# sloisel/LinearAlgebraMPI.jl

Hardware: AMD Instinct MI355X
Metric: SpMV GFLOP/s (2*nnz/t), 2-D 5-pt Poisson, fp64 (higher is better)
Workload: dtype f64

## Files before the change

include/hpcla_rocm.h:

```cpp
#ifndef HPCLA_ROCM_H
#define HPCLA_ROCM_H

#include <stdint.h>

#ifdef __cplusplus
extern "C" {
#endif

#define HPCLA_VERSION 100

#define HPCLA_OK 0
#define HPCLA_ERR_INVALID -1
#define HPCLA_ERR_HIP -2
#define HPCLA_ERR_RCCL -3
#define HPCLA_ERR_NO_DEVICE -4
#define HPCLA_ERR_UNSUPPORTED -5
#define HPCLA_ERR_ALLOC -6

#define HPCLA_LAYOUT_ROW 0
#define HPCLA_LAYOUT_COL 1

typedef struct hpcla_comm hpcla_comm_t;
typedef struct hpcla_halo_plan hpcla_halo_plan_t;

// ... 332 lines not shown
int64_t hpcla_cols16_padded_len(int64_t nnz);
int hpcla_cols16_encode_i32(const int32_t *rowptr, const int32_t *colval_split, int64_t nrows, int64_t nnz, int64_t n_own,
                            int index_base, const int32_t *block_list, int64_t n_blocks, int16_t *cols16,
                            int *ineligible_dev, void *stream);
int hpcla_spmv_cols16_f64_i32(const int32_t *rowptr, const int16_t *cols16, const double *nzval, const double *x, double *y,
                              int64_t nrows, int64_t nnz, int index_base, const int32_t *block_list, int64_t n_blocks,
                              void *stream);
int hpcla_spmv_dist_cols16_f64_i32(hpcla_halo_plan_t *plan, const int32_t *rowptr, const int32_t *colval_split,
                                   const int16_t *cols16, const double *nzval, const double *x, int64_t n_own, double *y,
                                   int64_t nrows, int64_t nnz, int index_base, const int32_t *interior_blocks,
                                   int64_t n_interior, const int32_t *boundary_blocks, int64_t n_boundary, void *stream);
int hpcla_spmv_dist_dot_cols16_f64_i32(hpcla_halo_plan_t *plan, hpcla_comm_t *comm, const int32_t *rowptr,
                                       const int32_t *colval_split, const int16_t *cols16, const double *nzval,
                                       const double *x, int64_t n_own, double *y, int64_t nrows, int64_t nnz,
                                       int index_base, const int32_t *interior_blocks, int64_t n_interior,
                                       const int32_t *boundary_blocks, int64_t n_boundary, double *dot_out_dev,
                                       void *work, void *stream);
int hpcla_spmv_tune_block_order_cols16_f64_i32(const int32_t *rowptr, const int16_t *cols16, const double *nzval,
                                               const double *x_own, double *y_scratch, int64_t nrows, int64_t nnz,
                                               int index_base, int64_t block_base, int64_t n_blocks, void *stream,
                                               int *chosen_group);

#define HPCLA_BLOCK_PATTERNS_WEAK_HASH 1
typedef struct hpcla_block_patterns hpcla_block_patterns_t;
int hpcla_block_patterns_create_i32(hpcla_block_patterns_t **out, const int32_t *rowptr, const int16_t *cols16, int64_t nrows,
                                    int64_t nnz, int index_base, const int32_t *block_list, int64_t block_base,
                                    int64_t n_blocks, int flags, void *stream);
int hpcla_block_patterns_destroy(hpcla_block_patterns_t *p);
int hpcla_block_patterns_info(const hpcla_block_patterns_t *p, int64_t *n_patterns, int64_t *table_bytes,
                              int64_t *n_candidates, int64_t *n_patterned);
int hpcla_spmv_patterns_f64_i32(const int32_t *rowptr, const int16_t *cols16, const hpcla_block_patterns_t *patterns,
                                const double *nzval, const double *x, double *y, int64_t nrows, int64_t nnz, int index_base,
                                const int32_t *block_list, int64_t n_blocks, void *stream);
int hpcla_spmv_dist_patterns_f64_i32(hpcla_halo_plan_t *plan, const int32_t *rowptr, const int32_t *colval_split,
                                     const int16_t *cols16, const hpcla_block_patterns_t *patterns, const double *nzval,
                                     const double *x, int64_t n_own, double *y, int64_t nrows, int64_t nnz, int index_base,
                                     const int32_t *interior_blocks, int64_t n_interior, const int32_t *boundary_blocks,
                                     int64_t n_boundary, void *stream);
int hpcla_spmv_dist_dot_patterns_f64_i32(hpcla_halo_plan_t *plan, hpcla_comm_t *comm, const int32_t *rowptr,
                                         const int32_t *colval_split, const int16_t *cols16,
                                         const hpcla_block_patterns_t *patterns, const double *nzval, const double *x,
                                         int64_t n_own, double *y, int64_t nrows, int64_t nnz, int index_base,
                                         const int32_t *interior_blocks, int64_t n_interior,
                                         const int32_t *boundary_blocks, int64_t n_boundary, double *dot_out_dev, void *work,
                                         void *stream);
int hpcla_spmv_tune_block_order_patterns_f64_i32(const int32_t *rowptr, const int16_t *cols16,
                                                 const hpcla_block_patterns_t *patterns, const double *nzval,
                                                 const double *x_own, double *y_scratch, int64_t nrows, int64_t nnz,
                                                 int index_base, int64_t block_base, int64_t n_blocks, void *stream,
                                                 int *chosen_group);

typedef struct hpcla_packed hpcla_packed_t;
int hpcla_packed_create_i32(hpcla_packed_t **out, const int32_t *rowptr, const int32_t *colval_split,
// ... 176 lines not shown
```

linearalgebrampi.jl_amd/_capi.py:

```python
from __future__ import annotations

import ctypes
import os

_HERE = os.path.dirname(os.path.abspath(__file__))
LIB_PATH = os.path.join(_HERE, "libhpcla_rocm.so")

OK = 0
LAYOUT_ROW = 0
LAYOUT_COL = 1
UNIQUE_ID_BYTES = 128
WINDOW_DESC_BYTES = 128
WINDOW_TABLE_ROWS = 4
COMM_NO_RCCL = 1
HALO_SINGLE_BUFFER = 1
BLOCK_PATTERNS_WEAK_HASH = 1


class HPCLAError(RuntimeError):
    def __init__(self, fn: str, status: int, text: str):
        super().__init__(f"{fn} failed with status {status}: {text}")
        self.status = status


_lib = None

_i32 = ctypes.c_int
_i64 = ctypes.c_int64
_u64 = ctypes.c_uint64
_f64 = ctypes.c_double
_f32 = ctypes.c_float
_vp = ctypes.c_void_p

_SIGNATURES = {
    "hpcla_version": [],
    "hpcla_last_error": [],
    "hpcla_device_count": [_vp],
    "hpcla_set_device": [_i32],
    "hpcla_device_info": [_i32, _vp, _vp, _i32],
    "hpcla_spmv_csr_f64_i32": [_vp, _vp, _vp, _vp, _vp, _i64, _i64, _i32, _vp],
    "hpcla_spmv_csr_f64_i64": [_vp, _vp, _vp, _vp, _vp, _i64, _i64, _i32, _vp],
    "hpcla_spmv_split_f64_i32": [_vp, _vp, _vp, _vp, _vp, _i64, _vp, _i64, _i64, _i32, _vp, _i64, _vp],
    "hpcla_spmv_split_f64_i64": [_vp, _vp, _vp, _vp, _vp, _i64, _vp, _i64, _i64, _i32, _vp, _i64, _vp],
    "hpcla_spmv_rows_per_block": [],
    "hpcla_spmv_longrows_work_bytes": [_i64],
    "hpcla_spmv_longrows_f64_i32": [_vp, _vp, _vp, _vp, _vp, _i64, _vp, _i64, _i64, _i32, _vp, _i64, _i64, _vp, _vp],
    "hpcla_spmv_longrows_f64_i64": [_vp, _vp, _vp, _vp, _vp, _i64, _vp, _i64, _i64, _i32, _vp, _i64, _i64, _vp, _vp],
    "hpcla_spmv_block_order_hint": [_vp, _i32],
    "hpcla_spmv_tune_block_order_f64_i32": [_vp, _vp, _vp, _vp, _vp, _i64, _vp, _i64, _i64, _i32, _vp, _vp],
    "hpcla_spmv_tune_block_order_f64_i64": [_vp, _vp, _vp, _vp, _vp, _i64, _vp, _i64, _i64, _i32, _vp, _vp],
    "hpcla_spmv_tune_block_order_cols16_f64_i32": [_vp, _vp, _vp, _vp, _vp, _i64, _i64, _i32, _i64, _i64, _vp, _vp],
    "hpcla_cols16_padded_len": [_i64],
    "hpcla_cols16_encode_i32": [_vp, _vp, _i64, _i64, _i64, _i32, _vp, _i64, _vp, _vp, _vp],
    "hpcla_spmv_cols16_f64_i32": [_vp, _vp, _vp, _vp, _vp, _i64, _i64, _i32, _vp, _i64, _vp],
    "hpcla_block_patterns_create_i32": [_vp, _vp, _vp, _i64, _i64, _i32, _vp, _i64, _i64, _i32, _vp],
    "hpcla_block_patterns_destroy": [_vp],
    "hpcla_block_patterns_info": [_vp, _vp, _vp, _vp, _vp],
    "hpcla_spmv_patterns_f64_i32": [_vp, _vp, _vp, _vp, _vp, _vp, _i64, _i64, _i32, _vp, _i64, _vp],
    "hpcla_spmv_tune_block_order_patterns_f64_i32": [_vp, _vp, _vp, _vp, _vp, _vp, _i64, _i64, _i32, _i64, _i64, _vp, _vp],
    "hpcla_spmm_rows_per_block": [],
    "hpcla_spmm_runs_desc_bytes": [_i64],
    "hpcla_spmm_runs_build_i32": [_vp, _vp, _i64, _i64, _i32, _i64, _vp, _vp, _vp],
    "hpcla_spmm_runs_build_i64": [_vp, _vp, _i64, _i64, _i32, _i64, _vp, _vp, _vp],
    "hpcla_spmm_banded_blocks_i32": [_vp, _vp, _i64, _i64, _i32, _i64, _i32, _vp, _vp],
    "hpcla_spmm_banded_blocks_i64": [_vp, _vp, _i64, _i64, _i32, _i64, _i32, _vp, _vp],
    "hpcla_spmm_runs_k16_f64_i32": [_vp, _vp, _vp, _vp, _vp, _i64, _vp, _i64, _i64, _i32, _vp, _vp, _i64, _vp],
    "hpcla_spmm_runs_k16_f64_i64": [_vp, _vp, _vp, _vp, _vp, _i64, _vp, _i64, _i64, _i32, _vp, _vp, _i64, _vp],
    "hpcla_spmm_runs_colmajor_k16_f64_i32": [_vp, _vp, _vp, _vp, _i64, _vp, _i64, _i64, _vp, _i64, _i64, _i64, _i32, _vp, _vp, _i64, _vp],
    "hpcla_spmm_runs_colmajor_k16_f64_i64": [_vp, _vp, _vp, _vp, _i64, _vp, _i64, _i64, _vp, _i64, _i64, _i64, _i32, _vp, _vp, _i64, _vp],
    "hpcla_spmm_runs_colmajor_tune_block_order_f64_i32": [_vp, _vp, _vp, _vp, _i64, _vp, _i64, _i64, _vp, _i64, _i64, _i64, _i32, _vp, _vp, _i64, _vp, _vp],
    "hpcla_spmm_runs_colmajor_tune_block_order_f64_i64": [_vp, _vp, _vp, _vp, _i64, _vp, _i64, _i64, _vp, _i64, _i64, _i64, _i32, _vp, _vp, _i64, _vp, _vp],
    "hpcla_spmm_block_order_hint": [_vp, _i32],
    "hpcla_spmm_tune_block_order_f64_i32": [_vp, _vp, _vp, _vp, _i64, _vp, _i64, _i64, _vp, _i64, _i64, _i64, _i32, _i32,
                                            _vp, _i64, _vp, _vp],
    "hpcla_spmm_tune_block_order_f64_i64": [_vp, _vp, _vp, _vp, _i64, _vp, _i64, _i64, _vp, _i64, _i64, _i64, _i32, _i32,
                                            _vp, _i64, _vp, _vp],
    "hpcla_remap_i32": [_vp, _vp, _vp, _i64, _i32, _vp],
    "hpcla_remap_i64": [_vp, _vp, _vp, _i64, _i32, _vp],
    "hpcla_remap_i64_to_i32": [_vp, _vp, _vp, _i64, _i32, _vp],
    "hpcla_narrow_i64_to_i32": [_vp, _vp, _i64, _vp, _vp],
# ... 224 lines not shown
```

linearalgebrampi.jl_amd/csrc/patterns.h:

```cpp
#pragma once
#include "common.h"

namespace hpcla {

constexpr int PAT_RPB = 256;
constexpr int PAT_HEAD = 272;
constexpr int PAT_NR = 257, PAT_PHASE = 258, PAT_WAVE = 260;
constexpr int64_t PAT_TABLE_CAP_BYTES = 256 * 1024;
constexpr int64_t PAT_MAX_LEN = 65535;

struct alignas(8) PatRec {
    int32_t first;
    int32_t id;
};

struct PatArgs {
    const PatRec *rec;
    const int16_t *table;
};

}

struct hpcla_block_patterns {
    int64_t nrows = 0, nnz = 0, all_blocks = 0;
    int index_base = 0;
    hpcla::PatRec *rec = nullptr;
    int16_t *table = nullptr;
    int64_t table_bytes = 0, n_patterns = 0, n_candidates = 0, n_patterned = 0;
};
```

linearalgebrampi.jl_amd/csrc/patterns.hip:

```cpp
#include <algorithm>
#include <unordered_map>
#include <vector>

#include "patterns.h"

namespace hpcla {

__device__ __forceinline__ uint64_t pat_mix(uint64_t key, uint64_t v)
{
    uint64_t z = key * 0x9E3779B97F4A7C15ull + v * 0xC2B2AE3D27D4EB4Full + 0x165667B19E3779F9ull;
    z = (z ^ (z >> 30)) * 0xBF58476D1CE4E5B9ull;
    z = (z ^ (z >> 27)) * 0x94D049BB133111EBull;
    return z ^ (z >> 31);
}

struct PatMeta {
    int32_t first, len;
};

__device__ __forceinline__ int64_t pat_block(const int32_t *list, int64_t base, int64_t b) { return list ? (int64_t)list[b] : base + b; }

__global__ __launch_bounds__(PAT_RPB) void pat_hash_kernel(const int32_t *__restrict__ rowptr, const int16_t *__restrict__ cols16,
                                                           int64_t nrows, int64_t nnz, int base, const int32_t *__restrict__ list,
                                                           int64_t run_base, int weak, uint64_t *__restrict__ hash,
// ... 51 lines not shown
                                                             PatRec *__restrict__ rec)
{
    const int64_t blk = pat_block(list, run_base, blockIdx.x);
    const PatRec rc = rec[blk];
    if (rc.id < 0) return;
    const int16_t *t = table + (int64_t)rc.id * 8;
    const int64_t r0 = blk * PAT_RPB;
    const int nr = (int)((nrows - r0) < PAT_RPB ? (nrows - r0) : PAT_RPB);
    const int64_t p0 = (int64_t)rowptr[r0] - base, len = (int64_t)rowptr[r0 + nr] - base - p0;
    const int phase = (int)(p0 & 7);
    int bad = (p0 != rc.first) | (t[PAT_NR] != (int16_t)nr) | (t[PAT_PHASE] != (int16_t)phase) | (len > PAT_MAX_LEN);
    if (!bad) {
        for (int i = threadIdx.x; i <= PAT_RPB; i += PAT_RPB)
            bad |= ((int64_t)(uint16_t)t[i] != (int64_t)rowptr[r0 + (i < nr ? i : nr)] - base - p0);
    }
    bad = __syncthreads_or(bad);
    if (!bad) {
        for (int64_t j = threadIdx.x; j < len; j += PAT_RPB) bad |= (t[PAT_HEAD + phase + j] != cols16[p0 + j]);
        bad = __syncthreads_or(bad);
    }
    if (bad && threadIdx.x == 0) rec[blk].id = -1;
}

static void patterns_free(hpcla_block_patterns *p)
{
    if (!p) return;
    if (p->rec) (void)hipFree(p->rec);
    if (p->table) (void)hipFree(p->table);
    delete p;
}

int patterns_args(const hpcla_block_patterns *p, int64_t nrows, int64_t nnz, int index_base, PatArgs *out)
{
    if (!p || !out) return set_error(HPCLA_ERR_INVALID, "block patterns: null handle");
    if (p->nrows != nrows || p->nnz != nnz || p->index_base != index_base)
        return set_error(HPCLA_ERR_INVALID, "block patterns: the handle was created for another structure (nrows / nnz / index_base)");
    out->rec = p->rec;
    out->table = p->table;
    return HPCLA_OK;
}

}

using namespace hpcla;

HPCLA_API int hpcla_block_patterns_create_i32(hpcla_block_patterns_t **out, const int32_t *rowptr, const int16_t *cols16,
                                              int64_t nrows, int64_t nnz, int index_base, const int32_t *block_list,
                                              int64_t block_base, int64_t n_blocks, int flags, void *stream)
{
    if (!out) return set_error(HPCLA_ERR_INVALID, "block_patterns_create: null out");
    *out = nullptr;
    if (nrows < 0 || nnz < 0) return set_error(HPCLA_ERR_INVALID, "block_patterns_create: negative size");
    if (index_base != 0 && index_base != 1) return set_error(HPCLA_ERR_INVALID, "block_patterns_create: index_base must be 0 or 1");
    if (flags & ~HPCLA_BLOCK_PATTERNS_WEAK_HASH) return set_error(HPCLA_ERR_INVALID, "block_patterns_create: unknown flag");
    const int64_t all_blocks = (nrows + PAT_RPB - 1) / PAT_RPB;
    int64_t nc = all_blocks, run_base = 0;
    if (block_list) {
        if (n_blocks < 0 || n_blocks > all_blocks) return set_error(HPCLA_ERR_INVALID, "block_patterns_create: n_blocks out of range");
        nc = n_blocks;
    } else if (block_base >= 0) {
        if (n_blocks < 0 || block_base + n_blocks > all_blocks)
            return set_error(HPCLA_ERR_INVALID, "block_patterns_create: block run out of bounds");
        nc = n_blocks;
        run_base = block_base;
    }
    if (nc == 0 || nnz == 0) return HPCLA_OK;
    if (!rowptr || !cols16) return set_error(HPCLA_ERR_INVALID, "block_patterns_create: null array");
    HPCLA_CHECK_GRID(nc, "block_patterns_create");
    hipStream_t s = as_stream(stream);

    uint64_t *d_hash = nullptr;
    PatMeta *d_meta = nullptr;
    PatRec *d_reps = nullptr;
    hpcla_block_patterns *p = nullptr;
    auto fail = [&](int code) {
        if (d_hash) (void)hipFree(d_hash);
        if (d_meta) (void)hipFree(d_meta);
        if (d_reps) (void)hipFree(d_reps);
        patterns_free(p);
        return code;
    };
#define PT_HIP(expr)                                                                                                   \
    do {                                                                                                               \
        hipError_t _e = (expr);                                                                                        \
        if (_e != hipSuccess) return fail(set_error(HPCLA_ERR_HIP, "%s failed: %s", #expr, hipGetErrorString(_e)));    \
    } while (0)
    PT_HIP(hipMalloc((void **)&d_hash, nc * sizeof(uint64_t)));
    PT_HIP(hipMalloc((void **)&d_meta, nc * sizeof(PatMeta)));
    pat_hash_kernel<<<(uint32_t)nc, PAT_RPB, 0, s>>>(rowptr, cols16, nrows, nnz, index_base, block_list, run_base,
                                                     (flags & HPCLA_BLOCK_PATTERNS_WEAK_HASH) ? 1 : 0, d_hash, d_meta);
    PT_HIP(hipGetLastError());
    std::vector<uint64_t> hash(nc);
    std::vector<PatMeta> meta(nc);
    std::vector<int32_t> blocks;
    PT_HIP(hipMemcpyAsync(hash.data(), d_hash, nc * sizeof(uint64_t), hipMemcpyDeviceToHost, s));
    PT_HIP(hipMemcpyAsync(meta.data(), d_meta, nc * sizeof(PatMeta), hipMemcpyDeviceToHost, s));
    if (block_list) {
        blocks.resize(nc);
// ... 34 lines not shown
    if (covered * 2 < nc || reps.empty()) return fail(HPCLA_OK);

    p = new hpcla_block_patterns;
    p->nrows = nrows; p->nnz = nnz; p->all_blocks = all_blocks; p->index_base = index_base;
    p->table_bytes = used * (int64_t)sizeof(int16_t);
    p->n_patterns = (int64_t)reps.size();
    p->n_candidates = nc;
    std::vector<PatRec> rec(all_blocks, PatRec{0, -1});
    for (int64_t b = 0; b < nc; ++b) {
        auto it = hash[b] == ~(uint64_t)0 ? kept.end() : kept.find(hash[b]);
        rec[block_of(b)] = PatRec{meta[b].first, it == kept.end() ? -1 : it->second};
    }
    PT_HIP(hipMalloc((void **)&p->rec, all_blocks * sizeof(PatRec)));
    PT_HIP(hipMalloc((void **)&p->table, p->table_bytes));
    PT_HIP(hipMalloc((void **)&d_reps, reps.size() * sizeof(PatRec)));
    PT_HIP(hipMemsetAsync(p->table, 0, p->table_bytes, s));
    PT_HIP(hipMemcpyAsync(p->rec, rec.data(), all_blocks * sizeof(PatRec), hipMemcpyHostToDevice, s));
    PT_HIP(hipMemcpyAsync(d_reps, reps.data(), reps.size() * sizeof(PatRec), hipMemcpyHostToDevice, s));
    pat_build_kernel<<<(uint32_t)reps.size(), PAT_RPB, 0, s>>>(rowptr, cols16, nrows, index_base, d_reps, p->table);
    PT_HIP(hipGetLastError());
    pat_verify_kernel<<<(uint32_t)nc, PAT_RPB, 0, s>>>(rowptr, cols16, nrows, index_base, block_list, run_base, p->table, p->rec);
    PT_HIP(hipGetLastError());
    PT_HIP(hipMemcpyAsync(rec.data(), p->rec, all_blocks * sizeof(PatRec), hipMemcpyDeviceToHost, s));
    PT_HIP(hipStreamSynchronize(s));
#undef PT_HIP
    for (const PatRec &r : rec) p->n_patterned += r.id >= 0;
    if (p->n_patterned * 2 < nc) return fail(HPCLA_OK);
    (void)hipFree(d_hash); (void)hipFree(d_meta); (void)hipFree(d_reps);
    *out = p;
    return HPCLA_OK;
}

HPCLA_API int hpcla_block_patterns_destroy(hpcla_block_patterns_t *p)
{
    patterns_free(p);
    return HPCLA_OK;
}

HPCLA_API int hpcla_block_patterns_info(const hpcla_block_patterns_t *p, int64_t *n_patterns, int64_t *table_bytes,
                                        int64_t *n_candidates, int64_t *n_patterned)
{
    if (!p) return set_error(HPCLA_ERR_INVALID, "block_patterns_info: null handle");
    if (n_patterns) *n_patterns = p->n_patterns;
    if (table_bytes) *table_bytes = p->table_bytes;
    if (n_candidates) *n_candidates = p->n_candidates;
    if (n_patterned) *n_patterned = p->n_patterned;
    return HPCLA_OK;
}
```

linearalgebrampi.jl_amd/csrc/spmv.hip:

```cpp
#include <stdlib.h>
#include <string.h>

#include <atomic>
#include <mutex>
#include <type_traits>
#include <unordered_map>

#include "common.h"
#include "halo_wait.h"
#include "patterns.h"

namespace hpcla {

constexpr int RPB = 256;
static_assert(RPB == PAT_RPB, "the pattern table is built for this kernel's row blocks");
constexpr int CHUNK = RPB * 8;
constexpr int UNROLL = CHUNK / RPB;

template <typename T, int N>
using vec = T __attribute__((ext_vector_type(N)));

struct Cols16 {};
struct Pat16 {};
template <typename P>
struct IndexPolicy {
    using row_t = P;
    using col_t = P;
    static constexpr int VEC = 4;
    static constexpr bool PATTERNS = false;
    static __device__ __forceinline__ int64_t decode(col_t c, int base, int64_t ) { return (int64_t)(P)(c - (P)base); }
    static __device__ __forceinline__ col_t fill(int base) { return (P)base; }
};
template <>
struct IndexPolicy<Cols16> {
    using row_t = int32_t;
    using col_t = int16_t;
    static constexpr int VEC = 8;
    static constexpr bool PATTERNS = false;
    static __device__ __forceinline__ int64_t decode(col_t d, int , int64_t r0) { return r0 + (int)d; }
    static __device__ __forceinline__ col_t fill(int ) { return 0; }
};
template <>
struct IndexPolicy<Pat16> : IndexPolicy<Cols16> {
    static constexpr bool PATTERNS = true;
};

template <bool SPLIT>
__device__ __forceinline__ double gather_x(const double *__restrict__ x_own,
                                           const double *__restrict__ x_ghost, int64_t n_own,
                                           int64_t col)
{
    if (SPLIT) {
        const double *p = col < n_own ? x_own + col : x_ghost + (col - n_own);
        return *p;
    }
    return x_own[col];
}

struct BlockSel {
    const int32_t *list;
    int64_t base;
    const int32_t *first_list;
    int64_t first_base;
    int64_t n_first;
    int64_t n_run;
    int32_t group_log2;
    int32_t nt_y;
// ... 18 lines not shown
            if (bs.first_list) return (int64_t)bs.first_list[b];
            return bs.first_base + (bs.group_log2 > 0 ? xcd_group_index(b, bs.n_run, bs.group_log2) : b);
        }
        wait = true;
        return bs.list ? (int64_t)bs.list[b - bs.n_first] : bs.base + (b - bs.n_first);
    }
    if (bs.list) return (int64_t)bs.list[b];
    return bs.base + (bs.group_log2 > 0 ? xcd_group_index(b, bs.n_run, bs.group_log2) : b);
}

__device__ __forceinline__ void block_dot_epilogue(double *s_scratch, double *__restrict__ dot_partial,
                                                   int64_t blk, double v)
{
#pragma unroll
    for (int off = 32; off > 0; off >>= 1) v += __shfl_down(v, off, 64);
    const int lane = threadIdx.x & 63, w = threadIdx.x >> 6;
    if (lane == 0) s_scratch[w] = v;
    __syncthreads();
    if (threadIdx.x == 0) dot_partial[blk] = ((s_scratch[0] + s_scratch[1]) + s_scratch[2]) + s_scratch[3];
}

constexpr int RG_CHW = 464;
constexpr int RG_UR = 8;

template <typename I, bool SPLIT, bool WAIT, bool LONGR = false>
__global__ __launch_bounds__(RPB) void spmv_rowgather_kernel(
    const typename IndexPolicy<I>::row_t *__restrict__ rowptr, const typename IndexPolicy<I>::col_t *__restrict__ colval,
    const double *__restrict__ nzval, const double *__restrict__ x_own, const double *x_ghost, int64_t n_own,
    double *__restrict__ y, int64_t nrows, int64_t nnz, int base,
    BlockSel bs, double *__restrict__ dot_partial, HaloWait hw, PushArgs push, int64_t long_min = 0, PatArgs pat = PatArgs{nullptr, nullptr})
{
    using IP = IndexPolicy<I>;
    using R = typename IP::row_t;
    using C = typename IP::col_t;
    constexpr int V = IP::VEC;
    constexpr int NV = (RG_CHW / V + 63) / 64;
    static_assert(!LONGR || !WAIT, "the long-row form is a plain launch");
    static_assert(V * sizeof(C) == 16 || sizeof(C) == 8, "one 16-byte column load per staged vector (Int64: two)");
    static_assert(RG_CHW % V == 0 && RG_CHW >= 64 * 7 + V - 1, "a pass holds a 7-entry stencil's wave behind any aligned start");
    __shared__ __attribute__((aligned(16))) C s_col_all[(RPB / 64) * RG_CHW];
    __shared__ __attribute__((aligned(16))) double s_val_all[(RPB / 64) * RG_CHW];
    __shared__ double s_red[RPB / 64];

    if constexpr (WAIT) {
        if ((int)blockIdx.x < push.n_blocks) {
            halo_push_block<R, RPB>(push, (int)blockIdx.x);
            return;
        }
    }
    const int tid = threadIdx.x;
    bool wait_ghosts;
    const int64_t blk = select_block<WAIT>(bs, wait_ghosts, WAIT ? push.n_blocks : 0);
    uint32_t waited = 0;
// ... 2 lines not shown
        x_ghost = hw.ghost0 + (int64_t)(waited & ~HALO_WAIT_TIMED_OUT) * hw.buf_stride;
    }
    const int64_t r0 = blk * RPB;
    const int nr = (int)((nrows - r0) < RPB ? (nrows - r0) : RPB);
    if (WAIT && (waited & HALO_WAIT_TIMED_OUT)) {
        if ((int)threadIdx.x < nr) y[r0 + threadIdx.x] = halo_poison();
        if (dot_partial && threadIdx.x == 0) dot_partial[blk] = halo_poison();
        return;
    }

    const int wave = __builtin_amdgcn_readfirstlane(tid >> 6), lane = tid & 63;
    C *s_col = s_col_all + wave * RG_CHW;
    double *s_val = s_val_all + wave * RG_CHW;
    const int64_t rw = r0 + wave * 64;
    const int nrw = nr - wave * 64 < 0 ? 0 : (nr - wave * 64 > 64 ? 64 : nr - wave * 64);
    double acc = 0.0, x_row = 0.0;
    if (nrw > 0) {
        const int ll = lane < nrw ? lane : nrw - 1;
        int64_t p0 = 0, p1 = 0;
        R rlo = 0, rhi = 0;
        const C *cols = colval;
        bool streamed = true;
        R roff = 0;
        if constexpr (IP::PATTERNS) {
            const int64_t rc64 = *reinterpret_cast<const int64_t *>(pat.rec + blk);
            const PatRec rc{(int32_t)rc64, (int32_t)(rc64 >> 32)};
            if (rc.id >= 0) {
                const int16_t *t = pat.table + (int64_t)rc.id * 8;
                const int32_t *wb = reinterpret_cast<const int32_t *>(t + PAT_WAVE) + wave;
                p0 = (int64_t)rc.first + wb[0];
                p1 = (int64_t)rc.first + wb[1];
                struct __attribute__((packed, aligned(2))) Pair { uint32_t v; };
                rlo = (R)reinterpret_cast<const Pair *>(t + wave * 64 + ll)->v;
                roff = rc.first + base;
                cols = t + PAT_HEAD - (rc.first & ~7);
                streamed = false;
            }
        }
        if (streamed) {
            p0 = (int64_t)rowptr[rw] - base;
            p1 = (int64_t)rowptr[rw + nrw] - base;
            rlo = rowptr[rw + ll];
            rhi = rowptr[rw + ll + 1];
        }
        const int64_t pa = p0 & ~(int64_t)(V - 1);
        const int64_t total = p1 - pa;
        if (dot_partial) x_row = x_own[rw + ll];
        const bool is_long = LONGR && lane < nrw && (int64_t)rhi - (int64_t)rlo >= long_min;
        for (int64_t c = 0; c < total; c += RG_CHW) {
            if (LONGR) {
                const int64_t lo_rel = (int64_t)rlo - base - pa, hi_rel = (int64_t)rhi - base - pa;
                const uint64_t covers = __ballot(is_long && lo_rel <= c && hi_rel >= c + RG_CHW);
                if (covers) {
                    const int64_t hi_l = __shfl(hi_rel, __ffsll((unsigned long long)covers) - 1, 64);
                    c = (hi_l / RG_CHW) * RG_CHW - RG_CHW;
                    continue;
                }
            }
            const int n = (int)((total - c) < RG_CHW ? (total - c) : RG_CHW);
            if (pa + c + ((n + V - 1) & ~(V - 1)) <= nnz) {
                const int last = (n - 1) & ~(V - 1);
                vec<C, V> cq[NV];
                vec<double, 2> va[NV][V / 2];
#pragma unroll
                for (int u = 0; u < NV; ++u) {
                    const int e0 = (u * 64 + lane) * V;
                    const int ee = e0 < last ? e0 : last;
                    cq[u] = *reinterpret_cast<const vec<C, V> *>(cols + pa + c + ee);
#pragma unroll
                    for (int k = 0; k < V / 2; ++k)
                        va[u][k] = *reinterpret_cast<const vec<double, 2> *>(nzval + pa + c + ee + 2 * k);
                }
// ... 315 lines not shown
    } else if (block_base >= 0) {
        if (n_blocks < 0 || block_base + n_blocks > all_blocks)
            return set_error(HPCLA_ERR_INVALID, "spmv: block range out of bounds");
        launch_blocks = n_blocks;
    } else {
        block_base = 0;
    }
    if (launch_blocks == 0) return HPCLA_OK;
    if (launch_blocks > 0x7fffffffLL) return set_error(HPCLA_ERR_INVALID, "spmv: too many blocks");
    dim3 grid((uint32_t)launch_blocks), block(RPB);
    hipStream_t s = as_stream(stream);
    if (split && !x_ghost) split = false;
    using IP = IndexPolicy<I>;
    const bool aligned = (reinterpret_cast<uintptr_t>(colval) % (IP::VEC * sizeof(typename IP::col_t)) == 0) &&
                         (reinterpret_cast<uintptr_t>(nzval) % 32 == 0);
    const BlockSel bs{block_list, block_base, nullptr, 0, 0, launch_blocks, block_list ? 0 : block_order_of(rowptr),
                      spmv_nt_y(dot_partial != nullptr)};
    HaloWait nowait;
    memset(&nowait, 0, sizeof(nowait));
    PushArgs nopush;
    memset(&nopush, 0, sizeof(nopush));
    if constexpr (std::is_same<I, Cols16>::value) {
        if (!aligned) return set_error(HPCLA_ERR_INVALID, "spmv: 16-bit columns need a 16-byte aligned copy and 32-byte aligned nzval");
        if (pat)
            spmv_rowgather_kernel<Pat16, false, false><<<grid, block, 0, s>>>(
                rowptr, colval, nzval, x_own, nullptr, 0, y, nrows, nnz, index_base, bs, dot_partial, nowait, nopush, 0, *pat);
        else
            spmv_rowgather_kernel<Cols16, false, false><<<grid, block, 0, s>>>(
                rowptr, colval, nzval, x_own, nullptr, 0, y, nrows, nnz, index_base, bs, dot_partial, nowait, nopush);
    } else if (aligned) {
        if (split)
            spmv_rowgather_kernel<I, true, false><<<grid, block, 0, s>>>(
                rowptr, colval, nzval, x_own, x_ghost, n_own, y, nrows, nnz, index_base, bs, dot_partial, nowait, nopush);
        else
            spmv_rowgather_kernel<I, false, false><<<grid, block, 0, s>>>(
                rowptr, colval, nzval, x_own, nullptr, 0, y, nrows, nnz, index_base, bs, dot_partial, nowait, nopush);
    } else {
        if (split)
            spmv_rowblock_kernel<I, true, false><<<grid, block, 0, s>>>(
                rowptr, colval, nzval, x_own, x_ghost, n_own, y, nrows, index_base, bs, dot_partial, nowait, nopush);
        else
            spmv_rowblock_kernel<I, false, false><<<grid, block, 0, s>>>(
                rowptr, colval, nzval, x_own, nullptr, 0, y, nrows, index_base, bs, dot_partial, nowait, nopush);
    }
    HPCLA_CHECK_LAUNCH();
    return HPCLA_OK;
}
// ... 118 lines not shown
                    double *dot_partial, int64_t block_base, const hpcla_block_patterns *patterns)
{
    PatArgs pa;
    if (patterns)
        if (const int rc = patterns_args(patterns, nrows, nnz, index_base, &pa)) return rc;
    return spmv_launch<Cols16>(rowptr, cols16, nzval, x, nullptr, 0, false, y, nrows, nnz, index_base, bl, nb, stream,
                               dot_partial, block_base, patterns ? &pa : nullptr);
}

}

using namespace hpcla;

HPCLA_API int hpcla_spmv_rows_per_block(void) { return RPB; }

static void set_block_order(const void *rowptr, int group_log2)
{
    std::lock_guard<std::mutex> lock(g_order_mu);
    if (group_log2 <= 0) g_order.erase(rowptr);
    else g_order[rowptr] = group_log2;
    g_order_count.store((int)g_order.size(), std::memory_order_relaxed);
}

template <typename I>
static int tune_block_order(const typename IndexPolicy<I>::row_t *rowptr, const typename IndexPolicy<I>::col_t *colval_split,
                            const double *nzval, const double *x_own,
                            const double *x_ghost, int64_t n_own, double *y_scratch, int64_t nrows, int64_t nnz,
                            int index_base, void *stream, int *chosen_group, int64_t run_base = -1, int64_t run_blocks = 0,
                            const PatArgs *pat = nullptr)
{
    if (chosen_group) *chosen_group = 1;
    if (nrows < 0 || nnz < 0 || !rowptr) return set_error(HPCLA_ERR_INVALID, "spmv_tune_block_order: bad arguments");
    set_block_order(rowptr, 0);
    const int64_t n_blocks = (nrows + RPB - 1) / RPB;
    if (n_blocks < 4096 || nnz == 0) return HPCLA_OK;
    if (run_base >= 0 && (run_blocks <= 0 || run_base + run_blocks > n_blocks))
        return run_blocks == 0 ? HPCLA_OK : set_error(HPCLA_ERR_INVALID, "spmv_tune_block_order: block run out of bounds");
    if (!y_scratch) return set_error(HPCLA_ERR_INVALID, "spmv_tune_block_order: null scratch vector");
    constexpr int NC = 4, ROUNDS = 4, REPS = 4;
    const int cand[NC] = {0, 3, 5, 6};
    float ms[NC][ROUNDS];
    hipEvent_t e0, e1;
    HPCLA_CHECK_HIP(hipEventCreate(&e0));
    HPCLA_CHECK_HIP(hipEventCreate(&e1));
    hipStream_t s = as_stream(stream);
    int rc = HPCLA_OK;
    for (int r = 0; r < ROUNDS && rc == HPCLA_OK; ++r)
        for (int c = 0; c < NC && rc == HPCLA_OK; ++c) {
            set_block_order(rowptr, cand[c]);
            if (hipEventRecord(e0, s) != hipSuccess) { rc = set_error(HPCLA_ERR_HIP, "spmv_tune_block_order: event"); break; }
            for (int i = 0; i < REPS && rc == HPCLA_OK; ++i)
                rc = spmv_launch<I>(rowptr, colval_split, nzval, x_own, x_ghost, n_own, true, y_scratch, nrows, nnz,
                                    index_base, nullptr, run_base >= 0 ? run_blocks : 0, stream, nullptr, run_base, pat);
            if (rc != HPCLA_OK) break;
            if (hipEventRecord(e1, s) != hipSuccess || hipEventSynchronize(e1) != hipSuccess ||
                hipEventElapsedTime(&ms[c][r], e0, e1) != hipSuccess)
                rc = set_error(HPCLA_ERR_HIP, "spmv_tune_block_order: timing");
        }
    (void)hipEventDestroy(e0);
    (void)hipEventDestroy(e1);
    set_block_order(rowptr, 0);
    if (rc != HPCLA_OK) return rc;
    float best_t[NC];
    for (int c = 0; c < NC; ++c) {
        float a = ms[c][1], b = ms[c][2], d = ms[c][3];
        best_t[c] = a > b ? (b > d ? b : (a > d ? d : a)) : (a > d ? a : (b > d ? d : b));
    }
    int best = 0;
    for (int c = 1; c < NC; ++c)
        if (best_t[c] < best_t[best]) best = c;
    if (best != 0 && best_t[best] > 0.99f * best_t[0]) best = 0;
    set_block_order(rowptr, cand[best]);
    if (chosen_group) *chosen_group = 1 << cand[best];
    return HPCLA_OK;
}

HPCLA_API int hpcla_spmv_tune_block_order_f64_i32(const int32_t *rowptr, const int32_t *colval_split, const double *nzval,
                                                  const double *x_own, const double *x_ghost, int64_t n_own,
                                                  double *y_scratch, int64_t nrows, int64_t nnz, int index_base,
                                                  void *stream, int *chosen_group)
{
    return tune_block_order<int32_t>(rowptr, colval_split, nzval, x_own, x_ghost, n_own, y_scratch, nrows, nnz, index_base,
                                     stream, chosen_group);
}

HPCLA_API int hpcla_spmv_tune_block_order_f64_i64(const int64_t *rowptr, const int64_t *colval_split, const double *nzval,
                                                  const double *x_own, const double *x_ghost, int64_t n_own,
                                                  double *y_scratch, int64_t nrows, int64_t nnz, int index_base,
                                                  void *stream, int *chosen_group)
{
    return tune_block_order<int64_t>(rowptr, colval_split, nzval, x_own, x_ghost, n_own, y_scratch, nrows, nnz, index_base,
                                     stream, chosen_group);
}

// ... 273 lines not shown
```

linearalgebrampi.jl_amd/sparse.py:

```python
from __future__ import annotations

import ctypes
from dataclasses import dataclass, field
from typing import Dict, List, Optional, Tuple

import numpy as np

from . import _capi
from .backends import (CommSerial, HPCBackend, assert_backends_compatible, attach_halo_windows, comm_allgather,
                       comm_alltoall_counts, comm_barrier, comm_exchange_indices, comm_rank, comm_size,
                       create_halo_plan, halo_ghost_ptr, halo_timed_out, require_device)
from .partition import (compute_partition_hash, compute_structural_hash, owner_of,
                        uniform_partition)
from .vectors import HPCVector, current_stream_ptr, dptr


import os as _os

_PACKED_BY_ENV = _os.environ.get("HPCLA_SPMV_PACKED", "") == "1"


def _torch():
    import torch
    return torch
# ... 101 lines not shown
            lo, hi = cut(cnt, c), cut(cnt, c + 1)
            chunk_of[off + lo:off + hi] = c
            newpos[off + lo:off + hi] = fill[c] + np.arange(hi - lo, dtype=np.int64)
            fill[c] += hi - lo
        off += cnt
    return send_chunks, recv_chunk_counts, chunk_of, newpos


INT32_MAX = int(np.iinfo(np.int32).max)


def narrowing_enabled() -> bool:
    return _os.environ.get("HPCLA_NARROW_INDICES", "1").strip().lower() not in ("0", "off", "false", "no")


def narrow_cols_enabled() -> bool:
    return _os.environ.get("HPCLA_NARROW_COLS", "1").strip().lower() not in ("0", "off", "false", "no")


def block_patterns_enabled() -> bool:
    return narrow_cols_enabled() and _os.environ.get("HPCLA_BLOCK_PATTERNS", "1").strip().lower() not in ("0", "off", "false", "no")


def create_block_patterns(rowptr_dev, cols16, nrows: int, nnz: int, block_list, block_base: int, n_blocks: int, flags: int = 0):
    h = ctypes.c_void_p()
    _capi.call("hpcla_block_patterns_create_i32", ctypes.byref(h), dptr(rowptr_dev), dptr(cols16), nrows, nnz, 0,
               dptr(block_list) if block_list is not None else None, block_base, n_blocks, flags, current_stream_ptr())
    return h if h else None


def block_patterns_info(handle) -> dict:
    v = [ctypes.c_int64() for _ in range(4)]
    _capi.call("hpcla_block_patterns_info", handle, *[ctypes.byref(c) for c in v])
    return dict(zip(("patterns", "table_bytes", "candidates", "patterned"), (int(c.value) for c in v)))


def encode_cols16(rowptr_dev, colval_split, nrows: int, nnz: int, n_own: int, block_list, n_blocks: int):
    torch = _torch()
    dev = colval_split.device
    out = torch.empty(_capi.load().hpcla_cols16_padded_len(nnz), dtype=torch.int16, device=dev)
    bad = torch.empty(1, dtype=torch.int32, device=dev)
    _capi.call("hpcla_cols16_encode_i32", dptr(rowptr_dev), dptr(colval_split), nrows, nnz, n_own, 0,
               dptr(block_list) if block_list is not None else None, n_blocks, dptr(out), dptr(bad), current_stream_ptr())
    return None if int(bad.item()) else out


def can_narrow_indices(nnz: int, nrows_local: int, n_own: int, n_ghost: int, index_base: int = 0) -> bool:
    lim = INT32_MAX - int(index_base)
    return (int(nnz) <= lim and int(nrows_local) <= lim and int(n_own) + int(n_ghost) <= lim and int(n_own) <= lim)


def split_colval(A: "HPCSparseMatrix", cmap: np.ndarray, to_i32: bool):
    torch = _torch()
    dev = A.backend.torch_device
    a64 = A.Ti == np.dtype(np.int64)
    out64 = a64 and not to_i32
    cmap_dev = torch.from_numpy(cmap.astype(np.int64 if out64 else np.int32)).to(dev)
# ... 57 lines not shown

        self.interior = self.boundary = None
        self.n_interior = self.n_boundary = 0
        if self.has_halo and A.nrows_local > 0:
            rpb = _capi.load().hpcla_spmv_rows_per_block()
            nblk = (A.nrows_local + rpb - 1) // rpb
            flags = torch.empty(nblk, dtype=torch.int32, device=dev)
            _capi.call(f"hpcla_classify_blocks_{sfx}", dptr(self.rowptr_of(A)), dptr(self.colval_split),
                       A.nrows_local, 0, self.n_own, rpb, dptr(flags), s)
            self.interior = torch.nonzero(flags == 0).flatten().to(torch.int32).contiguous()
            self.boundary = torch.nonzero(flags != 0).flatten().to(torch.int32).contiguous()
            self.n_interior = int(self.interior.numel())
            self.n_boundary = int(self.boundary.numel())
        self._keep = cmap_dev
        self.cols16 = None
        if (narrow_cols_enabled() and not self.is_i64 and not self.is_f32 and A.nrows_local > 0 and A.nnz > 0
                and (not self.has_halo or self.n_interior > 0)):
            self.cols16 = encode_cols16(self.rowptr_of(A), self.colval_split, A.nrows_local, A.nnz, self.n_own,
                                        self.interior if self.has_halo else None, self.n_interior if self.has_halo else 0)
        self.patterns = None
        if self.cols16 is not None and block_patterns_enabled():
            self.patterns = create_block_patterns(self.rowptr_of(A), self.cols16, A.nrows_local, A.nnz,
                                                  self.interior if self.has_halo else None, -1,
                                                  self.n_interior if self.has_halo else 0)
        self.block_group = 1
        self.block_group_measured = False
        want = _os.environ.get("HPCLA_BLOCK_ORDER", "auto").strip().lower()
        if want.isdigit():
            g = int(want)
            if g > 1024 or (g & (g - 1)) != 0:
                import sys
                sys.stderr.write(f"hpcla: HPCLA_BLOCK_ORDER={want} is not a power of two <= 1024; natural order\n")
                g = 1
            self.block_group = max(1, g)
        elif (want != "natural" and not self.is_f32 and A.nrows_local > 0 and A.nnz > 0
              and int(x.v.numel()) >= max(self.n_own, 1)):
            scratch = torch.empty(A.nrows_local, dtype=torch.float64, device=dev)
            ghost, _ng = self.ghost_tensor_ptr()
            chosen = ctypes.c_int(1)
            run = None
            if self.cols16 is not None and A.nzval.data_ptr() % 32 == 0:
                if not self.has_halo:
                    run = (-1, 0)
                else:
                    first, last = int(self.interior[0]), int(self.interior[-1])
                    if last - first + 1 == self.n_interior:
                        run = (first, self.n_interior)
# ... 36 lines not shown
    def timed_out(self) -> bool:
        return halo_timed_out(self.halo)

    def destroy(self) -> None:
        if getattr(self, "patterns", None) is not None:
            _capi.call("hpcla_block_patterns_destroy", self.patterns)
            self.patterns = None
        if self.halo:
            _capi.call("hpcla_halo_plan_destroy", self.halo)
            self.halo = ctypes.c_void_p()


_vector_plan_cache: Dict[tuple, VectorPlan] = {}


def get_vector_plan(A: "HPCSparseMatrix", x: HPCVector) -> VectorPlan:
    key = (A._ensure_hash(), x.structural_hash, str(A.T), str(A.Ti), "ROCArray")
    if A.Ti == np.dtype(np.int64) and not narrowing_enabled():
        key += ("wide",)
    if not narrow_cols_enabled():
        key += ("cols32",)
    elif not block_patterns_enabled():
        key += ("nopat",)
    plan = _vector_plan_cache.get(key)
    if plan is None:
        plan = VectorPlan(A, x)
        plan.key = key
        _vector_plan_cache[key] = plan
    if getattr(plan if plan.narrowed else A, "_block_order_hint", 1) != plan.block_group:
        _hint_block_order(A, plan)
    A._block_order_hint = plan.block_group
    return plan


def _unhint_block_order(ptr: int) -> None:
    try:
        _capi.load().hpcla_spmv_block_order_hint(ctypes.c_void_p(ptr), 0)
    except Exception:
        pass


def _unhint_spmm_block_order(ptr: int) -> None:
    try:
        _capi.load().hpcla_spmm_block_order_hint(ctypes.c_void_p(ptr), 0)
    except Exception:
        pass
# ... 510 lines not shown
```

Measured before the change: 1014.

## Add per-row column records for short block patterns in SpMV row-gather

```diff
diff --git a/include/hpcla_rocm.h b/include/hpcla_rocm.h
--- a/include/hpcla_rocm.h
+++ b/include/hpcla_rocm.h
@@ -378,6 +378,7 @@
                                                int *chosen_group);
 
 #define HPCLA_BLOCK_PATTERNS_WEAK_HASH 1
+#define HPCLA_BLOCK_PATTERNS_NO_ROWS 2
 typedef struct hpcla_block_patterns hpcla_block_patterns_t;
 int hpcla_block_patterns_create_i32(hpcla_block_patterns_t **out, const int32_t *rowptr, const int16_t *cols16, int64_t nrows,
                                     int64_t nnz, int index_base, const int32_t *block_list, int64_t block_base,
@@ -385,6 +386,7 @@
 int hpcla_block_patterns_destroy(hpcla_block_patterns_t *p);
 int hpcla_block_patterns_info(const hpcla_block_patterns_t *p, int64_t *n_patterns, int64_t *table_bytes,
                               int64_t *n_candidates, int64_t *n_patterned);
+int hpcla_block_patterns_rows_info(const hpcla_block_patterns_t *p, int64_t *n_row_patterns, int64_t *row_bytes);
 int hpcla_spmv_patterns_f64_i32(const int32_t *rowptr, const int16_t *cols16, const hpcla_block_patterns_t *patterns,
                                 const double *nzval, const double *x, double *y, int64_t nrows, int64_t nnz, int index_base,
                                 const int32_t *block_list, int64_t n_blocks, void *stream);
diff --git a/linearalgebrampi.jl_amd/_capi.py b/linearalgebrampi.jl_amd/_capi.py
--- a/linearalgebrampi.jl_amd/_capi.py
+++ b/linearalgebrampi.jl_amd/_capi.py
@@ -15,6 +15,7 @@
 COMM_NO_RCCL = 1
 HALO_SINGLE_BUFFER = 1
 BLOCK_PATTERNS_WEAK_HASH = 1
+BLOCK_PATTERNS_NO_ROWS = 2
 
 
 class HPCLAError(RuntimeError):
@@ -56,6 +57,7 @@
     "hpcla_block_patterns_create_i32": [_vp, _vp, _vp, _i64, _i64, _i32, _vp, _i64, _i64, _i32, _vp],
     "hpcla_block_patterns_destroy": [_vp],
     "hpcla_block_patterns_info": [_vp, _vp, _vp, _vp, _vp],
+    "hpcla_block_patterns_rows_info": [_vp, _vp, _vp],
     "hpcla_spmv_patterns_f64_i32": [_vp, _vp, _vp, _vp, _vp, _vp, _i64, _i64, _i32, _vp, _i64, _vp],
     "hpcla_spmv_tune_block_order_patterns_f64_i32": [_vp, _vp, _vp, _vp, _vp, _vp, _i64, _i64, _i32, _i64, _i64, _vp, _vp],
     "hpcla_spmm_rows_per_block": [],
diff --git a/linearalgebrampi.jl_amd/csrc/patterns.h b/linearalgebrampi.jl_amd/csrc/patterns.h
--- a/linearalgebrampi.jl_amd/csrc/patterns.h
+++ b/linearalgebrampi.jl_amd/csrc/patterns.h
@@ -5,9 +5,13 @@
 
 constexpr int PAT_RPB = 256;
 constexpr int PAT_HEAD = 272;
-constexpr int PAT_NR = 257, PAT_PHASE = 258, PAT_WAVE = 260;
+constexpr int PAT_NR = 257, PAT_PHASE = 258, PAT_WAVE = 260, PAT_ROWS = 270;
 constexpr int64_t PAT_TABLE_CAP_BYTES = 256 * 1024;
 constexpr int64_t PAT_MAX_LEN = 65535;
+constexpr int PAT_ROW_K = 8;
+constexpr int PAT_PASS = 464;
+constexpr int64_t PAT_ROWS_PATTERN_BYTES = (int64_t)PAT_RPB * PAT_ROW_K * 2;
+constexpr int64_t PAT_ROWS_CAP_BYTES = 256 * 1024;
 
 struct alignas(8) PatRec {
     int32_t first;
@@ -17,6 +21,7 @@
 struct PatArgs {
     const PatRec *rec;
     const int16_t *table;
+    const int16_t *rows;
 };
 
 }
@@ -26,5 +31,7 @@
     int index_base = 0;
     hpcla::PatRec *rec = nullptr;
     int16_t *table = nullptr;
+    int16_t *rows = nullptr;
+    int64_t n_row_patterns = 0;
     int64_t table_bytes = 0, n_patterns = 0, n_candidates = 0, n_patterned = 0;
 };
diff --git a/linearalgebrampi.jl_amd/csrc/patterns.hip b/linearalgebrampi.jl_amd/csrc/patterns.hip
--- a/linearalgebrampi.jl_amd/csrc/patterns.hip
+++ b/linearalgebrampi.jl_amd/csrc/patterns.hip
@@ -97,9 +97,35 @@
     if (bad && threadIdx.x == 0) rec[blk].id = -1;
 }
 
+__global__ __launch_bounds__(PAT_RPB) void pat_rows_kernel(int16_t *__restrict__ table, const int32_t *__restrict__ place,
+                                                           const int32_t *__restrict__ which, int16_t *__restrict__ rows)
+{
+    const int32_t w = which[blockIdx.x];
+    if (w < 0) return;
+    int16_t *t = table + (int64_t)place[blockIdx.x] * 8;
+    const int i = threadIdx.x, nr = t[PAT_NR], phase = t[PAT_PHASE];
+    const int lo = (uint16_t)t[i], hi = (uint16_t)t[i + 1];
+    int16_t *r = rows + ((int64_t)w * PAT_RPB + i) * PAT_ROW_K;
+#pragma unroll
+    for (int u = 0; u < PAT_ROW_K; ++u) r[u] = (i < nr && lo + u < hi) ? t[PAT_HEAD + phase + lo + u] : (int16_t)0;
+    if (i == 0) *reinterpret_cast<int32_t *>(t + PAT_ROWS) = w + 1;
+}
+
+static bool pattern_is_short(const int16_t *t)
+{
+    const int phase = t[PAT_PHASE];
+    for (int i = 0; i < PAT_RPB; ++i)
+        if ((int)(uint16_t)t[i + 1] - (int)(uint16_t)t[i] > PAT_ROW_K) return false;
+    const int32_t *wb = reinterpret_cast<const int32_t *>(t + PAT_WAVE);
+    for (int w = 0; w < PAT_RPB / 64; ++w)
+        if (((wb[w] + phase) & 7) + (wb[w + 1] - wb[w]) > PAT_PASS) return false;
+    return true;
+}
+
 static void patterns_free(hpcla_block_patterns *p)
 {
     if (!p) return;
+    if (p->rows) (void)hipFree(p->rows);
     if (p->rec) (void)hipFree(p->rec);
     if (p->table) (void)hipFree(p->table);
     delete p;
@@ -112,6 +138,7 @@
         return set_error(HPCLA_ERR_INVALID, "block patterns: the handle was created for another structure (nrows / nnz / index_base)");
     out->rec = p->rec;
     out->table = p->table;
+    out->rows = p->rows;
     return HPCLA_OK;
 }
 
@@ -127,7 +154,7 @@
     *out = nullptr;
     if (nrows < 0 || nnz < 0) return set_error(HPCLA_ERR_INVALID, "block_patterns_create: negative size");
     if (index_base != 0 && index_base != 1) return set_error(HPCLA_ERR_INVALID, "block_patterns_create: index_base must be 0 or 1");
-    if (flags & ~HPCLA_BLOCK_PATTERNS_WEAK_HASH) return set_error(HPCLA_ERR_INVALID, "block_patterns_create: unknown flag");
+    if (flags & ~(HPCLA_BLOCK_PATTERNS_WEAK_HASH | HPCLA_BLOCK_PATTERNS_NO_ROWS)) return set_error(HPCLA_ERR_INVALID, "block_patterns_create: unknown flag");
     const int64_t all_blocks = (nrows + PAT_RPB - 1) / PAT_RPB;
     int64_t nc = all_blocks, run_base = 0;
     if (block_list) {
@@ -147,8 +174,10 @@
     uint64_t *d_hash = nullptr;
     PatMeta *d_meta = nullptr;
     PatRec *d_reps = nullptr;
+    int32_t *d_which = nullptr;
     hpcla_block_patterns *p = nullptr;
     auto fail = [&](int code) {
+        if (d_which) (void)hipFree(d_which);
         if (d_hash) (void)hipFree(d_hash);
         if (d_meta) (void)hipFree(d_meta);
         if (d_reps) (void)hipFree(d_reps);
@@ -229,11 +258,34 @@
     pat_verify_kernel<<<(uint32_t)nc, PAT_RPB, 0, s>>>(rowptr, cols16, nrows, index_base, block_list, run_base, p->table, p->rec);
     PT_HIP(hipGetLastError());
     PT_HIP(hipMemcpyAsync(rec.data(), p->rec, all_blocks * sizeof(PatRec), hipMemcpyDeviceToHost, s));
+    std::vector<int16_t> table;
+    if (!(flags & HPCLA_BLOCK_PATTERNS_NO_ROWS)) {
+        table.resize(used);
+        PT_HIP(hipMemcpyAsync(table.data(), p->table, p->table_bytes, hipMemcpyDeviceToHost, s));
+    }
     PT_HIP(hipStreamSynchronize(s));
-#undef PT_HIP
     for (const PatRec &r : rec) p->n_patterned += r.id >= 0;
     if (p->n_patterned * 2 < nc) return fail(HPCLA_OK);
+    if (!(flags & HPCLA_BLOCK_PATTERNS_NO_ROWS)) {
+        std::vector<int32_t> pw(2 * reps.size());
+        for (size_t k = 0; k < reps.size(); ++k) {
+            pw[k] = reps[k].id;
+            const bool take = (p->n_row_patterns + 1) * PAT_ROWS_PATTERN_BYTES <= PAT_ROWS_CAP_BYTES &&
+                              pattern_is_short(table.data() + (int64_t)reps[k].id * 8);
+            pw[reps.size() + k] = take ? (int32_t)p->n_row_patterns++ : -1;
+        }
+        if (p->n_row_patterns > 0) {
+            PT_HIP(hipMalloc((void **)&p->rows, p->n_row_patterns * PAT_ROWS_PATTERN_BYTES));
+            PT_HIP(hipMalloc((void **)&d_which, pw.size() * sizeof(int32_t)));
+            PT_HIP(hipMemcpyAsync(d_which, pw.data(), pw.size() * sizeof(int32_t), hipMemcpyHostToDevice, s));
+            pat_rows_kernel<<<(uint32_t)reps.size(), PAT_RPB, 0, s>>>(p->table, d_which, d_which + reps.size(), p->rows);
+            PT_HIP(hipGetLastError());
+            PT_HIP(hipStreamSynchronize(s));
+        }
+    }
+#undef PT_HIP
     (void)hipFree(d_hash); (void)hipFree(d_meta); (void)hipFree(d_reps);
+    if (d_which) (void)hipFree(d_which);
     *out = p;
     return HPCLA_OK;
 }
@@ -254,3 +306,11 @@
     if (n_patterned) *n_patterned = p->n_patterned;
     return HPCLA_OK;
 }
+
+HPCLA_API int hpcla_block_patterns_rows_info(const hpcla_block_patterns_t *p, int64_t *n_row_patterns, int64_t *row_bytes)
+{
+    if (!p) return set_error(HPCLA_ERR_INVALID, "block_patterns_rows_info: null handle");
+    if (n_row_patterns) *n_row_patterns = p->n_row_patterns;
+    if (row_bytes) *row_bytes = p->n_row_patterns * PAT_ROWS_PATTERN_BYTES;
+    return HPCLA_OK;
+}
diff --git a/linearalgebrampi.jl_amd/csrc/spmv.hip b/linearalgebrampi.jl_amd/csrc/spmv.hip
--- a/linearalgebrampi.jl_amd/csrc/spmv.hip
+++ b/linearalgebrampi.jl_amd/csrc/spmv.hip
@@ -22,12 +22,13 @@
 
 struct Cols16 {};
 struct Pat16 {};
+struct Pat16R {};
 template <typename P>
 struct IndexPolicy {
     using row_t = P;
     using col_t = P;
     static constexpr int VEC = 4;
-    static constexpr bool PATTERNS = false;
+    static constexpr bool PATTERNS = false, ROWS = false;
     static __device__ __forceinline__ int64_t decode(col_t c, int base, int64_t ) { return (int64_t)(P)(c - (P)base); }
     static __device__ __forceinline__ col_t fill(int base) { return (P)base; }
 };
@@ -36,13 +37,17 @@
     using row_t = int32_t;
     using col_t = int16_t;
     static constexpr int VEC = 8;
-    static constexpr bool PATTERNS = false;
+    static constexpr bool PATTERNS = false, ROWS = false;
     static __device__ __forceinline__ int64_t decode(col_t d, int , int64_t r0) { return r0 + (int)d; }
     static __device__ __forceinline__ col_t fill(int ) { return 0; }
 };
 template <>
 struct IndexPolicy<Pat16> : IndexPolicy<Cols16> {
     static constexpr bool PATTERNS = true;
+};
+template <>
+struct IndexPolicy<Pat16R> : IndexPolicy<Pat16> {
+    static constexpr bool ROWS = true;
 };
 
 template <bool SPLIT>
@@ -107,13 +112,14 @@
 
 constexpr int RG_CHW = 464;
 constexpr int RG_UR = 8;
+static_assert(RG_CHW == PAT_PASS && RG_UR == PAT_ROW_K, "the row records of a short pattern are cut for one pass and one gather step");
 
 template <typename I, bool SPLIT, bool WAIT, bool LONGR = false>
 __global__ __launch_bounds__(RPB) void spmv_rowgather_kernel(
     const typename IndexPolicy<I>::row_t *__restrict__ rowptr, const typename IndexPolicy<I>::col_t *__restrict__ colval,
     const double *__restrict__ nzval, const double *__restrict__ x_own, const double *x_ghost, int64_t n_own,
     double *__restrict__ y, int64_t nrows, int64_t nnz, int base,
-    BlockSel bs, double *__restrict__ dot_partial, HaloWait hw, PushArgs push, int64_t long_min = 0, PatArgs pat = PatArgs{nullptr, nullptr})
+    BlockSel bs, double *__restrict__ dot_partial, HaloWait hw, PushArgs push, int64_t long_min = 0, PatArgs pat = PatArgs{nullptr, nullptr, nullptr})
 {
     using IP = IndexPolicy<I>;
     using R = typename IP::row_t;
@@ -162,6 +168,7 @@
         const C *cols = colval;
         bool streamed = true;
         R roff = 0;
+        int32_t rowset = 0;
         if constexpr (IP::PATTERNS) {
             const int64_t rc64 = *reinterpret_cast<const int64_t *>(pat.rec + blk);
             const PatRec rc{(int32_t)rc64, (int32_t)(rc64 >> 32)};
@@ -170,6 +177,7 @@
                 const int32_t *wb = reinterpret_cast<const int32_t *>(t + PAT_WAVE) + wave;
                 p0 = (int64_t)rc.first + wb[0];
                 p1 = (int64_t)rc.first + wb[1];
+                if constexpr (IP::ROWS) rowset = *reinterpret_cast<const int32_t *>(t + PAT_ROWS);
                 struct __attribute__((packed, aligned(2))) Pair { uint32_t v; };
                 rlo = (R)reinterpret_cast<const Pair *>(t + wave * 64 + ll)->v;
                 roff = rc.first + base;
@@ -187,7 +195,46 @@
         const int64_t total = p1 - pa;
         if (dot_partial) x_row = x_own[rw + ll];
         const bool is_long = LONGR && lane < nrw && (int64_t)rhi - (int64_t)rlo >= long_min;
-        for (int64_t c = 0; c < total; c += RG_CHW) {
+        if constexpr (IP::ROWS) {
+            if (rowset > 0 && total > 0) {
+                const int n = (int)total;
+                const vec<C, RG_UR> rq =
+                    *reinterpret_cast<const vec<C, RG_UR> *>(pat.rows + ((int64_t)(rowset - 1) * RPB + tid) * RG_UR);
+                vec<int32_t, 4> rw4 = __builtin_bit_cast(vec<int32_t, 4>, rq);
+                double xx[RG_UR], vv[RG_UR];
+                int lo = 0, len = 0;
+                auto gathers = [&]() {
+                    asm volatile("" : "+v"(rlo), "+v"(rw4));
+                    const vec<C, RG_UR> d = __builtin_bit_cast(vec<C, RG_UR>, rw4);
+                    lo = (int)((int64_t)roff - base - pa) + (int)((uint32_t)rlo & 0xffffu);
+                    len = lane < nrw ? (int)((uint32_t)rlo >> 16) - (int)((uint32_t)rlo & 0xffffu) : 0;
+#pragma unroll
+                    for (int u = 0; u < RG_UR; ++u) { xx[u] = 0.0; if (u < len) xx[u] = x_own[r0 + (int)d[u]]; }
+                };
+                if (pa + ((n + V - 1) & ~(V - 1)) <= nnz) {
+                    const int last = (n - 1) & ~(V - 1);
+                    const int e0 = lane * V, ee = e0 < last ? e0 : last;
+                    vec<double, 2> va[V / 2];
+#pragma unroll
+                    for (int k = 0; k < V / 2; ++k) va[k] = *reinterpret_cast<const vec<double, 2> *>(nzval + pa + ee + 2 * k);
+                    gathers();
+                    if (e0 < n) {
+#pragma unroll
+                        for (int k = 0; k < V / 2; ++k) *reinterpret_cast<vec<double, 2> *>(&s_val[e0 + 2 * k]) = va[k];
+                    }
+                } else {
+                    gathers();
+                    for (int e = lane; e < n; e += 64) s_val[e] = pa + e < nnz ? nzval[pa + e] : 0.0;
+                }
+                __builtin_amdgcn_fence(__ATOMIC_RELEASE, "wavefront");
+                __builtin_amdgcn_wave_barrier();
+#pragma unroll
+                for (int u = 0; u < RG_UR; ++u) { vv[u] = 0.0; if (u < len) vv[u] = s_val[lo + u]; }
+#pragma unroll
+                for (int u = 0; u < RG_UR; ++u) if (u < len) acc += vv[u] * xx[u];
+            }
+        }
+        for (int64_t c = 0; c < (IP::ROWS && rowset > 0 ? 0 : total); c += RG_CHW) {
             if (LONGR) {
                 const int64_t lo_rel = (int64_t)rlo - base - pa, hi_rel = (int64_t)rhi - base - pa;
                 const uint64_t covers = __ballot(is_long && lo_rel <= c && hi_rel >= c + RG_CHW);
@@ -549,7 +596,10 @@
     memset(&nopush, 0, sizeof(nopush));
     if constexpr (std::is_same<I, Cols16>::value) {
         if (!aligned) return set_error(HPCLA_ERR_INVALID, "spmv: 16-bit columns need a 16-byte aligned copy and 32-byte aligned nzval");
-        if (pat)
+        if (pat && pat->rows)
+            spmv_rowgather_kernel<Pat16R, false, false><<<grid, block, 0, s>>>(
+                rowptr, colval, nzval, x_own, nullptr, 0, y, nrows, nnz, index_base, bs, dot_partial, nowait, nopush, 0, *pat);
+        else if (pat)
             spmv_rowgather_kernel<Pat16, false, false><<<grid, block, 0, s>>>(
                 rowptr, colval, nzval, x_own, nullptr, 0, y, nrows, nnz, index_base, bs, dot_partial, nowait, nopush, 0, *pat);
         else
@@ -714,6 +764,7 @@
     g_order_count.store((int)g_order.size(), std::memory_order_relaxed);
 }
 
+constexpr float TUNE_PAT_MARGIN = 0.03f;
 template <typename I>
 static int tune_block_order(const typename IndexPolicy<I>::row_t *rowptr, const typename IndexPolicy<I>::col_t *colval_split,
                             const double *nzval, const double *x_own,
@@ -759,9 +810,23 @@
         best_t[c] = a > b ? (b > d ? b : (a > d ? d : a)) : (a > d ? a : (b > d ? d : b));
     }
     int best = 0;
-    for (int c = 1; c < NC; ++c)
-        if (best_t[c] < best_t[best]) best = c;
-    if (best != 0 && best_t[best] > 0.99f * best_t[0]) best = 0;
+    if (pat) {
+        for (int c = 1; c < NC; ++c) {
+            bool every = true;
+            for (int r = 1; r < ROUNDS; ++r) every = every && ms[c][r] < ms[0][r];
+            if (every && best_t[c] <= (1.0f - TUNE_PAT_MARGIN) * best_t[0] && (best == 0 || best_t[c] < best_t[best])) best = c;
+        }
+    } else {
+        for (int c = 1; c < NC; ++c)
+            if (best_t[c] < best_t[best]) best = c;
+        if (best != 0 && best_t[best] > 0.99f * best_t[0]) best = 0;
+    }
+    if (const char *v = getenv("HPCLA_TUNE_VERBOSE"); v && atoi(v)) {
+        for (int c = 0; c < NC; ++c)
+            fprintf(stderr, "hpcla tune_block_order%s: groups of %d: rounds %.5f %.5f %.5f %.5f median %.5f\n", pat ? " (patterns)" : "",
+                    1 << cand[c], ms[c][0], ms[c][1], ms[c][2], ms[c][3], best_t[c]);
+        fprintf(stderr, "hpcla tune_block_order%s: chose groups of %d\n", pat ? " (patterns)" : "", 1 << cand[best]);
+    }
     set_block_order(rowptr, cand[best]);
     if (chosen_group) *chosen_group = 1 << cand[best];
     return HPCLA_OK;
diff --git a/linearalgebrampi.jl_amd/sparse.py b/linearalgebrampi.jl_amd/sparse.py
--- a/linearalgebrampi.jl_amd/sparse.py
+++ b/linearalgebrampi.jl_amd/sparse.py
@@ -147,6 +147,10 @@
     return narrow_cols_enabled() and _os.environ.get("HPCLA_BLOCK_PATTERNS", "1").strip().lower() not in ("0", "off", "false", "no")
 
 
+def pattern_rows_enabled() -> bool:
+    return _os.environ.get("HPCLA_PATTERN_ROWS", "1").strip().lower() not in ("0", "off", "false", "no")
+
+
 def create_block_patterns(rowptr_dev, cols16, nrows: int, nnz: int, block_list, block_base: int, n_blocks: int, flags: int = 0):
     h = ctypes.c_void_p()
     _capi.call("hpcla_block_patterns_create_i32", ctypes.byref(h), dptr(rowptr_dev), dptr(cols16), nrows, nnz, 0,
@@ -158,6 +162,12 @@
     v = [ctypes.c_int64() for _ in range(4)]
     _capi.call("hpcla_block_patterns_info", handle, *[ctypes.byref(c) for c in v])
     return dict(zip(("patterns", "table_bytes", "candidates", "patterned"), (int(c.value) for c in v)))
+
+
+def block_patterns_rows_info(handle) -> dict:
+    v = [ctypes.c_int64() for _ in range(2)]
+    _capi.call("hpcla_block_patterns_rows_info", handle, *[ctypes.byref(c) for c in v])
+    return dict(zip(("row_patterns", "row_bytes"), (int(c.value) for c in v)))
 
 
 def encode_cols16(rowptr_dev, colval_split, nrows: int, nnz: int, n_own: int, block_list, n_blocks: int):
@@ -261,7 +271,8 @@
         if self.cols16 is not None and block_patterns_enabled():
             self.patterns = create_block_patterns(self.rowptr_of(A), self.cols16, A.nrows_local, A.nnz,
                                                   self.interior if self.has_halo else None, -1,
-                                                  self.n_interior if self.has_halo else 0)
+                                                  self.n_interior if self.has_halo else 0,
+                                                  0 if pattern_rows_enabled() else _capi.BLOCK_PATTERNS_NO_ROWS)
         self.block_group = 1
         self.block_group_measured = False
         want = _os.environ.get("HPCLA_BLOCK_ORDER", "auto").strip().lower()
@@ -344,6 +355,8 @@
         key += ("cols32",)
     elif not block_patterns_enabled():
         key += ("nopat",)
+    elif not pattern_rows_enabled():
+        key += ("norows",)
     plan = _vector_plan_cache.get(key)
     if plan is None:
         plan = VectorPlan(A, x)
```

Result: no change. 1018 (median of 6 runs) (+0.4%).
